# Daniel-Starr/pointcloudhookup

Hardware: AMD Instinct MI355X
Metric: Mpts/s ground-filter+tower-cluster, 100 M-pt corridor; % HBM roofline on kNN (higher is better)
Workload: dtype f32 (filter) + f64 (distance predicate)

## Files before the change

### pointcloudhookup_amd/csrc/pch_dbscan.hip

```cpp
#include "pch_prims.h"

namespace pch {

constexpr int DB_THREADS = 256;
constexpr int DB_WAVES   = DB_THREADS / 64;
constexpr int DB_ROWS    = 25;
constexpr int INT_BIG    = 0x7fffffff;
constexpr int DB_FEW_QUERIES = 24;
constexpr int DB_AHEAD = 3;
constexpr long long DB_LONG_TOT = 8192;
constexpr int DB_SEGS = 43;

struct DbGrid {
    float   ox, oy, oz;
    double  cell;
    double  inv_cell;
    double  eps2;
    float   eps2_lo, eps2_hi;
    int     bx, by, bz;
    int     mx, my, mz;
    int64_t chunk_size;
    const uint32_t* chunk_bad;
    const uint32_t* chunk_cells;
    int     min_samples;
// ... 411 lines not shown
        float4 nxt[CS_ROUNDS];
        auto tile = [&](int t0, auto FULL_T) {
            constexpr bool FULL = decltype(FULL_T)::value;
            float4 row[CS_ROUNDS];
            uint32_t key[CS_ROUNDS], rank[CS_ROUNDS];
            const int seg = t0 + w * (64 * CS_ROUNDS);
#pragma unroll
            for (int r = 0; r < CS_ROUNDS; ++r) row[r] = nxt[r];
            if (t0 + CS_TILE < cn) fetch(t0 + CS_TILE, nxt);
#ifdef PCH_CS_STAMPS
            tlast = wall_clock64();
#endif
#pragma unroll
            for (int r = 0; r < CS_ROUNDS; ++r) {
                const bool valid = FULL || seg + r * 64 + l < cn;
                bool ok;
                key[r] = cs_cell_key(g, row[r].x, row[r].y, row[r].z, ok);
                const uint32_t d = (relkey(key[r]) >> shift) & mask;
                uint32_t np;
                const uint32_t rk = dbits <= 8 ? wave_match<8>(d, valid, np) : wave_match<9>(d, valid, np);
                const uint32_t prior = cnt[w][d];
                __builtin_amdgcn_wave_barrier();
                if (valid && rk == 0) cnt[w][d] = prior + np;
                __builtin_amdgcn_wave_barrier();
                rank[r] = prior + rk;
            }
            __syncthreads();
            CS_TILE_STAMP(0);
            if (tid < CS_BINS) {
                uint32_t run = base[tid];
#pragma unroll
                for (int w2 = 0; w2 < CS_WAVES; ++w2) {
                    const uint32_t cc = cnt[w2][tid];
                    off[w2][tid] = run;
                    cnt[w2][tid] = 0;
                    run += cc;
                }
                base[tid] = run;
            }
            __syncthreads();
            CS_TILE_STAMP(1);
#pragma unroll
            for (int r = 0; r < CS_ROUNDS; ++r) {
                if (FULL || seg + r * 64 + l < cn) {
                    const uint32_t d = (relkey(key[r]) >> shift) & mask;
                    const uint32_t pos = off[w][d] + rank[r];
                    dst[pos] = row[r];
                    if constexpr (LAST) keys_out[lo + pos] = hi | key[r];
                }
            }
            CS_TILE_STAMP(2);
        };
        fetch(0, nxt);
        int t0 = 0;
        for (; t0 + CS_TILE <= cn; t0 += CS_TILE) tile(t0, std::true_type{});
        if (t0 < cn) tile(t0, std::false_type{});
        __syncthreads();
        CS_STAMP();
    };
    for (int p = 0; p < passes; ++p) {
        const bool first = p == 0, last = p == passes - 1;
        if (first && last) run_pass(p, std::true_type{}, std::true_type{});
        else if (first)    run_pass(p, std::true_type{}, std::false_type{});
        else if (last)     run_pass(p, std::false_type{}, std::true_type{});
        else               run_pass(p, std::false_type{}, std::false_type{});
    }
#ifdef PCH_CS_STAMPS
    __syncthreads();
    CS_STAMP();
    if (stamps && blockIdx.x == gridDim.x / 2 && threadIdx.x == 0) for (int k = 0; k < 3; ++k) stamps[8 + k] = tacc[k];
#endif
}

constexpr int CT_SLOTS = 4096;
constexpr int CT_BITS  = 12;
constexpr int CT_CELLS = 1024;
constexpr uint32_t CT_EMPTY = 0xFFFFFFFFu;
static_assert(CT_SLOTS == 1 << CT_BITS && CT_CELLS + CS_THREADS < CT_SLOTS, "the table never fills (see sweep 1)");

__device__ __forceinline__ uint32_t ct_hash(uint32_t k) { return (k * 0x9E3779B1u) >> (32 - CT_BITS); }

__global__ __launch_bounds__(CS_THREADS) void db_cellscatter_k(
    const float* __restrict__ xyz, int64_t n, DbGrid g, uint32_t* __restrict__ bad, uint32_t* __restrict__ ovf,
    float4* __restrict__ pts, uint64_t* __restrict__ keys_out, uint32_t* __restrict__ status) {
    __shared__ uint32_t tkey[CT_SLOTS];
    __shared__ uint32_t tcnt[CT_SLOTS];
    __shared__ uint32_t skey[CT_CELLS];
    __shared__ uint32_t wsum[CS_WAVES];
    __shared__ uint32_t flags[5];
    const int tid = threadIdx.x, w = wave_id(), l = lane_id();
    const int64_t c = blockIdx.x;
    const int64_t lo = c * g.chunk_size;
    const int cn = (int)((n - lo) < g.chunk_size ? (n - lo) : g.chunk_size);
    const Row3* __restrict__ rows = reinterpret_cast<const Row3*>(xyz) + lo;
    for (int j = tid; j < CT_SLOTS; j += CS_THREADS) { tkey[j] = CT_EMPTY; tcnt[j] = 0u; }
    if (tid < 5) flags[tid] = 0u;
    __syncthreads();
    constexpr int HU = 8;
    for (int i0 = 0; i0 < cn; i0 += HU * CS_THREADS) {
        if (__hip_atomic_load(&flags[3], __ATOMIC_RELAXED, __HIP_MEMORY_SCOPE_WORKGROUP)) break;
        Row3 q[HU];
#pragma unroll
        for (int u = 0; u < HU; ++u) {
            const int i = i0 + u * CS_THREADS + tid;
            q[u] = rows[i < cn ? i : 0];
        }
#pragma unroll
        for (int u = 0; u < HU; ++u) {
            const bool in = i0 + u * CS_THREADS + tid < cn;
            const bool fin = fabsf(q[u].x) < INFINITY && fabsf(q[u].y) < INFINITY && fabsf(q[u].z) < INFINITY;
            bool ok;
            const uint32_t k = cs_cell_key(g, q[u].x, q[u].y, q[u].z, ok);
            if (in && !fin) flags[0] = 1u;
            else if (in && !ok) flags[1] = 1u;
            if (in && fin && __hip_atomic_load(&flags[3], __ATOMIC_RELAXED, __HIP_MEMORY_SCOPE_WORKGROUP) == 0u) {
                uint32_t h = ct_hash(k);
                for (int p = 0; p < CT_SLOTS; ++p, h = (h + 1u) & (CT_SLOTS - 1)) {
                    const uint32_t old = atomicCAS(&tkey[h], CT_EMPTY, k);
                    if (old == CT_EMPTY && atomicAdd(&flags[2], 1u) >= (uint32_t)CT_CELLS) flags[3] = 1u;
                    if (old == CT_EMPTY || old == k) { atomicAdd(&tcnt[h], 1u); break; }
                }
            }
        }
    }
    __syncthreads();
    const bool isbad = flags[0] != 0u;
    const uint32_t ncell = flags[2];
    const bool over = !isbad && ncell > (uint32_t)CT_CELLS;
    if (tid == 0) {
        ovf[c] = over ? 1u : 0u;
        if (!over) {
            bad[c] = isbad ? 1u : 0u;
            if (!isbad && flags[1]) atomicOr(status, 1u);
        }
    }
    if (over) return;
    const int sh = g.bx + g.by + g.bz;
    const uint64_t hi = sh < 64 ? ((uint64_t)c << sh) : 0ull;
    if (isbad || ncell == 1u) {
        for (int i = tid; i < cn; i += CS_THREADS) {
            const Row3 q = rows[i];
            float4 o4;
            o4.x = q.x; o4.y = q.y; o4.z = q.z; o4.w = __uint_as_float((uint32_t)(lo + i));
            pts[lo + i] = o4;
            bool ok;
            keys_out[lo + i] = isbad ? hi : (hi | cs_cell_key(g, q.x, q.y, q.z, ok));
        }
        return;
    }
    const int P = 1 << (32 - __clz((int)ncell - 1));
    for (int j0 = 0; j0 < CT_SLOTS; j0 += CS_THREADS) {
        const uint32_t k = tkey[j0 + tid];
        const uint64_t m = __ballot(k != CT_EMPTY);
        uint32_t base = 0;
        if (l == 0 && m) base = atomicAdd(&flags[4], (uint32_t)__popcll(m));
        base = (uint32_t)__shfl((int)base, 0, 64);
        if (k != CT_EMPTY) skey[base + (uint32_t)__popcll(m & lanemask_lt())] = k;
    }
    for (int j = (int)ncell + tid; j < P; j += CS_THREADS) skey[j] = CT_EMPTY;
    __syncthreads();
    for (int k = 2; k <= P; k <<= 1) {
        for (int j = k >> 1; j > 0; j >>= 1) {
            for (int t = tid; t < P / 2; t += CS_THREADS) {
                const int a = 2 * t - (t & (j - 1)), b = a + j;
                const uint32_t ka = skey[a], kb = skey[b];
                if ((ka > kb) == ((a & k) == 0)) { skey[a] = kb; skey[b] = ka; }
            }
            __syncthreads();
        }
    }
    {
        uint32_t slot[4], cnt[4], sum = 0;
#pragma unroll
        for (int u = 0; u < 4; ++u) {
            const int j = 4 * tid + u;
            slot[u] = 0; cnt[u] = 0;
            if (j < (int)ncell) {
                const uint32_t k = skey[j];
                uint32_t h = ct_hash(k);
                for (int p = 0; p < CT_SLOTS && tkey[h] != k; ++p) h = (h + 1u) & (CT_SLOTS - 1);
                slot[u] = h;
                cnt[u] = tcnt[h];
            }
            sum += cnt[u];
        }
        const uint32_t incl = wave_scan_incl(sum);
        if (l == 63) wsum[w] = incl;
        __syncthreads();
        uint32_t run = incl - sum;
        for (int w2 = 0; w2 < w; ++w2) run += wsum[w2];
#pragma unroll
        for (int u = 0; u < 4; ++u) {
            if (4 * tid + u < (int)ncell) tcnt[slot[u]] = run;
            run += cnt[u];
        }
    }
    __syncthreads();
    for (int i0 = 0; i0 < cn; i0 += HU * CS_THREADS) {
        Row3 q[HU];
#pragma unroll
        for (int u = 0; u < HU; ++u) {
            const int i = i0 + u * CS_THREADS + tid;
            q[u] = rows[i < cn ? i : 0];
        }
#pragma unroll
        for (int u = 0; u < HU; ++u) {
            const int i = i0 + u * CS_THREADS + tid;
            if (i < cn) {
                bool ok;
                const uint32_t k = cs_cell_key(g, q[u].x, q[u].y, q[u].z, ok);
                uint32_t h = ct_hash(k);
                for (int p = 0; p < CT_SLOTS && tkey[h] != k; ++p) h = (h + 1u) & (CT_SLOTS - 1);
                const uint32_t pos = atomicAdd(&tcnt[h], 1u);
                if (pos >= (uint32_t)cn) continue;
                float4 o4;
                o4.x = q[u].x; o4.y = q[u].y; o4.z = q[u].z; o4.w = __uint_as_float((uint32_t)(lo + i));
                pts[lo + pos] = o4;
                keys_out[lo + pos] = hi | k;
            }
        }
    }
}

constexpr int DC_ITEMS = SCAN_TILE / DB_THREADS;
static_assert(DC_ITEMS == 8, "two 64-byte key loads per thread");

__device__ __forceinline__ void dc_load_keys(const uint64_t* __restrict__ keys, int64_t base, int64_t n,
                                             uint64_t (&k)[DC_ITEMS], uint64_t& prev) {
    if (base + DC_ITEMS <= n) {
        const ulonglong2* q = reinterpret_cast<const ulonglong2*>(keys + base);
#pragma unroll
        for (int j = 0; j < DC_ITEMS / 2; ++j) { const ulonglong2 v = q[j]; k[2 * j] = v.x; k[2 * j + 1] = v.y; }
    } else {
#pragma unroll
        for (int j = 0; j < DC_ITEMS; ++j) k[j] = base + j < n ? keys[base + j] : 0ull;
    }
    prev = (base > 0 && base < n) ? keys[base - 1] : 0ull;
}

__global__ __launch_bounds__(DB_THREADS) void db_heads_k(const uint64_t* __restrict__ keys, int64_t n,
                                                         uint32_t* __restrict__ tile_sums) {
    __shared__ uint32_t wsum[DB_WAVES];
    const int64_t base = (int64_t)blockIdx.x * SCAN_TILE + (int64_t)threadIdx.x * DC_ITEMS;
    uint64_t k[DC_ITEMS], prev;
    dc_load_keys(keys, base, n, k, prev);
    uint32_t heads = 0;
#pragma unroll
    for (int j = 0; j < DC_ITEMS; ++j) {
        const int64_t i = base + j;
        heads += (i < n && (i == 0 || k[j] != (j ? k[j - 1] : prev))) ? 1u : 0u;
    }
    heads = wave_reduce_add(heads);
    if (lane_id() == 0) wsum[wave_id()] = heads;
    __syncthreads();
    if (threadIdx.x == 0) {
        uint32_t t = 0;
#pragma unroll
        for (int w = 0; w < DB_WAVES; ++w) t += wsum[w];
        tile_sums[blockIdx.x] = t;
    }
}

__global__ __launch_bounds__(DB_THREADS) void db_cells_k(const uint64_t* __restrict__ keys,
                                                         const uint32_t* __restrict__ tile_excl, int64_t n,
                                                         int sh, int64_t nchunks,
                                                         uint32_t* __restrict__ cid,
                                                         uint32_t* __restrict__ cell_start,
                                                         uint64_t* __restrict__ cell_key,
                                                         uint32_t* __restrict__ chunk_cells,
                                                         uint32_t* __restrict__ cell_acc) {
    __shared__ uint32_t wsum[DB_WAVES];
    const int64_t base = (int64_t)blockIdx.x * SCAN_TILE + (int64_t)threadIdx.x * DC_ITEMS;
    uint64_t k[DC_ITEMS], prev;
    dc_load_keys(keys, base, n, k, prev);
    bool hd[DC_ITEMS];
    uint32_t heads = 0;
// ... 18 lines not shown
            const uint64_t key = k[j], pk = j ? k[j - 1] : prev;
            cell_start[cc[j]] = (uint32_t)i;
            cell_key[cc[j]] = key;
            uint4* a4 = reinterpret_cast<uint4*>(cell_acc + 8 * (int64_t)cc[j]);
            a4[0] = make_uint4(0u, 0u, 0u, 0u);
            a4[1] = make_uint4(0u, 0u, 0u, 0u);
            const uint64_t ch = sh < 64 ? key >> sh : 0, pch = sh < 64 ? pk >> sh : 0;
            if (i == 0 || ch != pch) chunk_cells[ch] = cc[j];
        }
        if (i == n - 1) { cell_start[cc[j] + 1] = (uint32_t)n; chunk_cells[nchunks] = cc[j] + 1; }
    }
    if (base + DC_ITEMS <= n) {
        uint4* o = reinterpret_cast<uint4*>(cid + base);
        o[0] = make_uint4(cc[0], cc[1], cc[2], cc[3]);
        o[1] = make_uint4(cc[4], cc[5], cc[6], cc[7]);
    } else {
#pragma unroll
        for (int j = 0; j < DC_ITEMS; ++j)
            if (base + j < n) cid[base + j] = cc[j];
    }
}
struct RowSet {
    int ca[DB_ROWS], cb[DB_ROWS];
};

__device__ __forceinline__ int db_lower(const uint64_t* __restrict__ a, int m, uint64_t k) {
    int lo = 0, hi = m;
    while (lo < hi) { const int mid = (lo + hi) >> 1; if (a[mid] < k) lo = mid + 1; else hi = mid; }
    return lo;
}
__device__ __forceinline__ int2 db_row_run(const DbGrid& g, const uint64_t* __restrict__ cell_key, uint64_t key,
                                           int row) {
    const uint64_t cx = key & ((1ull << g.bx) - 1);
    const uint64_t cy = (key >> g.bx) & ((1ull << g.by) - 1);
    const uint64_t cz = (key >> (g.bx + g.by)) & ((1ull << g.bz) - 1);
    const int sh = g.bx + g.by + g.bz;
    const uint64_t chunk = sh < 64 ? (key >> sh) : 0;
    const int ny = (int)cy + DB_ROW_DY[row], nz = (int)cz + DB_ROW_DZ[row];
    int2 v;
    v.x = 0; v.y = 0;
    if (ny >= 0 && ny <= g.my && nz >= 0 && nz <= g.mz) {
        const int xlo = (int)cx - 2 < 0 ? 0 : (int)cx - 2;
        const int xhi = (int)cx + 2 > g.mx ? g.mx : (int)cx + 2;
        const int c0 = (int)g.chunk_cells[chunk], c1 = (int)g.chunk_cells[chunk + 1];
        v.x = c0 + db_lower(cell_key + c0, c1 - c0, db_pack(g, chunk, (uint64_t)nz, (uint64_t)ny, (uint64_t)xlo));
        const uint64_t khi = db_pack(g, chunk, (uint64_t)nz, (uint64_t)ny, (uint64_t)xhi);
        uint64_t kk[5];
#pragma unroll
        for (int i = 0; i < 5; ++i) kk[i] = v.x + i < c1 ? cell_key[v.x + i] : ~0ull;
        int cntx = 0;
#pragma unroll
        for (int i = 0; i < 5; ++i) cntx += kk[i] <= khi ? 1 : 0;
        v.y = v.x + cntx;
    }
    return v;
}

__device__ __forceinline__ void db_rows(const DbGrid& g, const uint64_t* __restrict__ cell_key, uint64_t key,
                                        RowSet* __restrict__ rs, const int2* __restrict__ rowtab, int cell) {
    const int l = lane_id();
    if (rowtab) {
        if (l < DB_ROWS) {
            const int2 v = rowtab[(int64_t)cell * DB_ROWS + l];
            rs->ca[l] = v.x;
            rs->cb[l] = v.y;
        }
        __builtin_amdgcn_wave_barrier();
        return;
    }
    if (l < DB_ROWS) {
        const int2 v = db_row_run(g, cell_key, key, l);
        rs->ca[l] = v.x;
        rs->cb[l] = v.y;
    }
    __builtin_amdgcn_wave_barrier();
}

__global__ __launch_bounds__(DB_THREADS) void db_rowtab_k(DbGrid g, const uint64_t* __restrict__ cell_key,
                                                          int m, int2* __restrict__ rowtab) {
    const int c = (blockIdx.x * DB_WAVES + wave_id()) * 2 + (lane_id() >> 5);
    const int l = lane_id() & 31;
    if (c >= m || l >= DB_ROWS) return;
    rowtab[(int64_t)c * DB_ROWS + l] = db_row_run(g, cell_key, cell_key[c], l);
}

template <bool COUNT>
__global__ __launch_bounds__(DB_THREADS) void db_core_k(DbGrid g, const float4* __restrict__ pts,
                                                        const uint32_t* __restrict__ cell_start,
                                                        const uint64_t* __restrict__ cell_key, int m,
                                                        const int2* __restrict__ rowtab,
                                                        uint8_t* __restrict__ core_s,
                                                        uint32_t* __restrict__ cell_ncore,
                                                        unsigned long long* __restrict__ stats) {
    unsigned long long n_useful = 0, n_slots = 0, n_tiles = 0;
    auto tally = [&]() {
        if (COUNT && lane_id() == 0) {
            atomicAdd(&stats[0], n_useful); atomicAdd(&stats[1], n_slots);
            atomicAdd(&stats[2], 1ull); atomicAdd(&stats[3], n_tiles);
        }
    };
    __shared__ RowSet rows[DB_WAVES];
    __shared__ DbPair tiles[DB_WAVES][32];
    __shared__ uint32_t seg_a[DB_WAVES][DB_SEGS], seg_b[DB_WAVES][DB_SEGS];
    const int c = blockIdx.x * DB_WAVES + wave_id();
    if (c >= m) return;
    const int l = lane_id();
    const uint32_t s = cell_start[c], e = cell_start[c + 1];
    const int cnt = (int)(e - s);
    {
        const int sh = g.bx + g.by + g.bz;
        if (g.chunk_bad[sh < 64 ? (cell_key[c] >> sh) : 0]) {
            for (uint32_t i = s + l; i < e; i += 64) core_s[i] = 0;
            if (l == 0) cell_ncore[c] = 0;
            return;
        }
    }
    if (cnt >= g.min_samples) {
        for (uint32_t i = s + l; i < e; i += 64) core_s[i] = 1;
        if (l == 0) cell_ncore[c] = (uint32_t)cnt;
        return;
    }
    RowSet* rs = &rows[wave_id()];
    db_rows(g, cell_key, cell_key[c], rs, rowtab, c);
    long long tot = 0;
    if (l < DB_ROWS) tot = (long long)cell_start[rs->cb[l]] - (long long)cell_start[rs->ca[l]];
    tot = wave_reduce_add(tot);
    if (tot < (long long)g.min_samples) {
        for (uint32_t i = s + l; i < e; i += 64) core_s[i] = 0;
        if (l == 0) cell_ncore[c] = 0;
        return;
    }
    uint32_t* sa = seg_a[wave_id()];
    uint32_t* sb = seg_b[wave_id()];
    {
        const uint64_t xmask = (1ull << g.bx) - 1;
        const int cx = (int)(cell_key[c] & xmask);
        if (l < DB_ROWS) {
            const int ca = rs->ca[l], cb = rs->cb[l];
            if (l < 9) {
                int ia = ca, ib = cb;
                if (ca < cb) {
                    if ((int)(cell_key[ca] & xmask) == cx - 2) ia = ca + 1;
                    if (ib > ia && (int)(cell_key[cb - 1] & xmask) == cx + 2) ib = cb - 1;
                }
                sa[l] = cell_start[ia];      sb[l] = cell_start[ib];
                sa[9 + l] = cell_start[ca];  sb[9 + l] = cell_start[ia];
                sa[18 + l] = cell_start[ib]; sb[18 + l] = cell_start[cb];
            } else {
                sa[18 + l] = cell_start[ca]; sb[18 + l] = cell_start[cb];
            }
        }
        __builtin_amdgcn_wave_barrier();
    }
    uint32_t ncore = 0;
    const bool long_sweep = tot >= DB_LONG_TOT;
    if (cnt < DB_FEW_QUERIES) {
        for (uint32_t q = s; q < e; ++q) {
            const float4 qp = pts[q];
            int count = 0;
            if (long_sweep) {
                for (int r = 0; r < DB_SEGS && count < g.min_samples; ++r) {
                    const uint32_t pa = sa[r], pb = sb[r];
                    for (uint32_t j0 = pa; j0 < pb && count < g.min_samples; j0 += 64u * DB_AHEAD) {
                        float4 P[DB_AHEAD];
#pragma unroll
                        for (int u = 0; u < DB_AHEAD; ++u) {
// ... 797 lines not shown
        }
    }
}

__global__ __launch_bounds__(DB_THREADS) void db_remap_points_k(const float4* __restrict__ pts,
                                                                const uint8_t* __restrict__ core_s, int64_t n,
                                                                const int32_t* __restrict__ map, int32_t nmap,
                                                                int32_t* __restrict__ labels) {
    const int64_t i = (int64_t)blockIdx.x * DB_THREADS + threadIdx.x;
    if (i >= n) return;
    const uint32_t o = __float_as_uint(pts[i].w);
    int32_t lab = -1;
    if (core_s[i]) {
        const int32_t old = labels[o];
        lab = (old >= 0 && old < nmap) ? map[old] : -1;
    }
    labels[o] = lab;
}
__global__ __launch_bounds__(DB_THREADS) void db_remap_cells_k(int* __restrict__ cell_label,
                                                               const uint32_t* __restrict__ cell_ncore, int m,
                                                               const int32_t* __restrict__ map, int32_t nmap) {
    const int c = blockIdx.x * DB_THREADS + threadIdx.x;
    if (c >= m) return;
    if (cell_ncore[c] == 0) return;
    const int old = cell_label[c];
    const int neu = (old >= 0 && old < nmap) ? map[old] : -1;
    cell_label[c] = neu >= 0 ? neu : INT_BIG;
}

__global__ __launch_bounds__(DB_THREADS) void db_first_rows_k(const uint32_t* __restrict__ bits,
                                                              const uint32_t* __restrict__ rank, int64_t nw,
                                                              int32_t* __restrict__ out) {
    const int64_t i = (int64_t)blockIdx.x * DB_THREADS + threadIdx.x;
    if (i >= nw) return;
    uint32_t b = bits[i];
    uint32_t c = rank[i];
    while (b) {
        const int t = __builtin_ctz(b);
        b &= b - 1;
        out[c++] = (int32_t)(i * 32 + t);
    }
}

__global__ __launch_bounds__(DB_THREADS) void db_strip_pairs_k(const float4* __restrict__ pts,
                                                               const uint32_t* __restrict__ cell_start,
                                                               const uint8_t* __restrict__ core_s,
                                                               const uint32_t* __restrict__ cell_ncore,
                                                               const float* __restrict__ cell_box,
                                                               const int* __restrict__ cell_label, int m, float x_lo,
                                                               float x_hi, int32_t cap, int32_t* __restrict__ out_pairs,
                                                               int32_t* __restrict__ out_count) {
    const int c = blockIdx.x * DB_WAVES + wave_id();
    if (c >= m) return;
    if (cell_ncore[c] == 0) return;
    if (!(cell_box[6 * (int64_t)c + 3] >= x_lo && cell_box[6 * (int64_t)c] < x_hi)) return;
    const int l = lane_id();
    const uint32_t a = cell_start[c], b = cell_start[c + 1];
    uint32_t best = 0xFFFFFFFFu;
    for (uint32_t i = a + l; i < b; i += 64) {
        if (!core_s[i]) continue;
        const float4 p = pts[i];
        if (p.x >= x_lo && p.x < x_hi) {
            const uint32_t row = __float_as_uint(p.w);
            best = row < best ? row : best;
        }
    }
    best = wave_reduce_min(best);
    if (l == 0 && best != 0xFFFFFFFFu) {
        const int32_t slot = atomicAdd(out_count, 1);
        if (slot < cap) {
            out_pairs[2 * slot] = (int32_t)best;
            out_pairs[2 * slot + 1] = cell_label[c];
        }
    }
}

__global__ void db_prelabel_k(const uint32_t* __restrict__ total, int32_t* __restrict__ out_nclusters,
                              uint32_t* __restrict__ box_acc, int64_t box_words) {
    if (threadIdx.x == 0 && blockIdx.x == 0) *out_nclusters = (int32_t)*total;
    const int64_t i = (int64_t)blockIdx.x * blockDim.x + threadIdx.x;
    if (box_acc && i < box_words) box_acc[i] = 0u;
}

struct DbWs {
    uint32_t* meta;
    uint64_t *k0, *k1, *cell_key;
    uint32_t *v0, *v1, *head, *cid, *cell_start, *cell_ncore, *flag, *radix_ws, *scan_ws;
    float4   *pts, *xbuf;
    uint8_t*  core_s;
    float*    cell_box;
    uint32_t* cell_acc;
    int*      cell_min;
    int      *parent, *root, *comp_min, *cell_label;
    int2*     rowtab;
    int64_t   rowtab_cells;
    uint32_t* chunk_bad;
    uint32_t* chunk_ovf;
    uint32_t* chunk_cells;
    uint32_t* comp;
    uint32_t* flag2;
    unsigned long long* core_stats;
    uint32_t* scan1_b;
};

static void db_plan(Arena& a, int64_t n, DbWs& w) {
    const int64_t nn = n > 0 ? n : 1;
    w.meta = a.take<uint32_t>(64);
    w.scan1_b = a.take<uint32_t>(scan1_ws_u32(nn / 32 + 1));
    w.chunk_cells = a.take<uint32_t>(nn + 8);
    w.core_stats = a.take<unsigned long long>(4);
    w.chunk_bad = a.take<uint32_t>(nn + 8);
    w.chunk_ovf = a.take<uint32_t>(nn + 8);
    w.k0 = a.take<uint64_t>(nn);
    w.k1 = a.take<uint64_t>(nn);
    w.v0 = a.take<uint32_t>(nn);
    w.v1 = a.take<uint32_t>(nn);
    w.head = a.take<uint32_t>(nn + 8);
    w.cid = a.take<uint32_t>(nn);
    w.pts = a.take<float4>(nn);
    w.xbuf = a.take<float4>(nn);
    w.core_s = a.take<uint8_t>(nn);
    w.cell_key = a.take<uint64_t>(nn);
    w.cell_start = a.take<uint32_t>(nn + 8);
    w.cell_ncore = a.take<uint32_t>(nn);
    w.cell_box = a.take<float>(6 * nn);
    w.cell_acc = a.take<uint32_t>(8 * nn);
    w.cell_min = a.take<int>(nn);
    w.parent = a.take<int>(nn);
    w.root = a.take<int>(nn);
    w.comp_min = a.take<int>(nn);
    w.cell_label = a.take<int>(nn);
    w.flag = a.take<uint32_t>(nn / 16 + 256);
    w.radix_ws = a.take<uint32_t>(radix_ws_u32(nn));
    w.scan_ws = a.take<uint32_t>(scan_ws_u32(nn));
    w.rowtab_cells = nn / 4 > 65536 ? nn / 4 : (nn < 65536 ? nn : 65536);
    w.rowtab = a.take<int2>((size_t)w.rowtab_cells * DB_ROWS);
    w.comp = a.take<uint32_t>(3 * nn);
    w.flag2 = a.take<uint32_t>(nn + 8);
}

struct DbCells {
    DbGrid g; const float4* pts; const uint32_t* cell_start; const uint64_t* cell_key; int m;
    const int2* rowtab;
    const uint8_t* core_s; const uint32_t* cell_ncore; const float* cell_box;
};
#define DB_GRID_ARGS(c) (c).g, (c).pts, (c).cell_start, (c).cell_key, (c).m, (c).rowtab
#define DB_CELL_ARGS(c) DB_GRID_ARGS(c), (c).core_s, (c).cell_ncore, (c).cell_box

struct DbTuning { int sort_mode; bool no_boxfold, no_xcd, count_pairs; };
static int g_sort_mode = -1;
static thread_local bool g_count_pairs = false;
static DbTuning db_tuning() {
    static const bool no_boxfold = getenv("PCH_DB_NO_BOXFOLD") != nullptr, no_xcd = getenv("PCH_DB_NO_XCD") != nullptr;
    int m = __atomic_load_n(&g_sort_mode, __ATOMIC_RELAXED);
    if (m < 0) {
        const char* e = getenv("PCH_DBSCAN_SORT");
        m = (e && strcmp(e, "chunk") == 0) ? 1 : (e && strcmp(e, "global") == 0) ? 2 : 0;
        __atomic_store_n(&g_sort_mode, m, __ATOMIC_RELAXED);
    }
    return {m, no_boxfold, no_xcd, g_count_pairs};
}

struct DbLastRun { void* ws; size_t ws_bytes; int64_t n; DbCells c; };
static thread_local DbLastRun g_last = {nullptr, 0, 0, {}};

void ws_touched(const void* base, size_t bytes) {
// ... 76 lines not shown
    g.eps2_lo = nextafterf((float)(g.eps2 * (1.0 - 1.0 / 1048576.0)), -INFINITY);
    g.eps2_hi = nextafterf((float)(g.eps2 * (1.0 + 1.0 / 1048576.0)), INFINITY);
    if (!(g.eps2_hi < 3.0e38f)) { g.eps2_lo = -1.0f; g.eps2_hi = NAN; }
    g.chunk_size = r.chunk_size;
    g.chunk_bad = r.w.chunk_bad;
    g.chunk_cells = r.w.chunk_cells;
    g.min_samples = min_samples;
    int mc[3] = {0, 0, 0};
    bool overflow = false;
    for (int k = 0; k < 3; ++k) {
        const double ext = ((double)box[3 + k] - (double)box[k]) * g.inv_cell;
        if (!(ext < 2.0e9)) overflow = true;
        else mc[k] = (int)ext + 1;
    }
    cellbits = db_cell_bits(g, mc[0], mc[1], mc[2]);
    nbits = cellbits + bits_for((uint64_t)r.nchunks);
    return overflow || nbits > 64;
}

static int db_run_chunks(const DbRun& r, double eps, int32_t min_samples, void* ws, size_t ws_bytes, int32_t* k_host) {
    int32_t offset = 0;
    for (int64_t c = 0; c < r.nchunks; ++c) {
        const int64_t lo = c * r.chunk_size, cn = (r.n - lo) < r.chunk_size ? (r.n - lo) : r.chunk_size;
        int32_t kc = 0;
        PCH_TRY(dbscan_run(r.xyz + 3 * lo, cn, eps, min_samples, 0, nullptr, r.labels + lo,
                           r.core ? r.core + lo : nullptr, r.out_nclusters, ws, ws_bytes, r.s, &kc));
        if (kc > 0 && offset > 0)
            PCH_LAUNCH("db_add_offset", db_add_offset_k, dim3((unsigned)ceil_div(cn, DB_THREADS)), dim3(DB_THREADS), 0,
                       r.s, r.labels + lo, cn, offset);
        offset += kc;
    }
    PCH_HIP_TRY(hipMemcpyAsync(r.out_nclusters, &offset, sizeof(int32_t), hipMemcpyHostToDevice, r.s));
    PCH_HIP_TRY(hipStreamSynchronize(r.s));
    if (k_host) *k_host = offset;
    g_last.ws = nullptr;
    return PCH_OK;
}

static int db_compress(const DbRun& r, DbGrid& g, int& cellbits, bool& done) {
    const DbWs& w = r.w; const hipStream_t s = r.s; const int64_t n = r.n;
    const unsigned gn = (unsigned)ceil_div(n, DB_THREADS);
    int64_t* first_bad = reinterpret_cast<int64_t*>(w.meta + 12);
    PCH_HIP_TRY(hipMemsetAsync(first_bad, 0xFF, sizeof(int64_t), s));
    PCH_LAUNCH("db_first_bad", db_first_bad_k, dim3(db_stride_blocks(n)), dim3(DB_THREADS), 0, s, r.xyz, n,
               reinterpret_cast<unsigned long long*>(first_bad));
    PCH_HIP_TRY(hipMemsetAsync(w.meta + 6, 0, 6 * sizeof(uint32_t), s));
    for (int axis = 0; axis < 3; ++axis) {
        PCH_LAUNCH("dbc_axis_keys", dbc_axis_keys_k, dim3(gn), dim3(DB_THREADS), 0, s, r.xyz, n, axis, w.k0, w.v0);
        PCH_TRY(radix_sort_pairs(w.k0, w.v0, w.k1, w.v1, n, 32, w.radix_ws, s));
        const bool in1 = radix_sort_result_buffer(32) == 1;
        const uint64_t* ksa = in1 ? w.k1 : w.k0;
        const uint32_t* vsa = in1 ? w.v1 : w.v0;
        PCH_LAUNCH("dbc_heads", dbc_heads_k, dim3(gn), dim3(DB_THREADS), 0, s, ksa, n, g.inv_cell, w.flag2);
        PCH_TRY(scan_exclusive_u32(w.flag2, w.head, n, w.scan_ws, nullptr, s));
        PCH_HIP_TRY(hipMemsetAsync(w.cell_start, 0, sizeof(uint32_t) * (size_t)(n + 8), s));
        for (int phase = 0; phase < 2; ++phase)
            PCH_LAUNCH("dbc_local", dbc_local_k, dim3(gn), dim3(DB_THREADS), 0, s, ksa, w.flag2, w.head, n, g.inv_cell,
                       w.cell_box, phase, w.cid, w.cell_start, w.meta + 6);
        PCH_TRY(scan_exclusive_u32(w.cell_start, w.cell_start, n, w.scan_ws, nullptr, s));
        PCH_LAUNCH("dbc_comp", dbc_comp_k, dim3(gn), dim3(DB_THREADS), 0, s, vsa, w.flag2, w.head, w.cid, w.cell_start,
                   n, axis, w.comp, w.meta + 9);
    }
    uint32_t back[8];
    PCH_HIP_TRY(hipMemcpyAsync(back, w.meta + 6, sizeof(back), hipMemcpyDeviceToHost, s));
    PCH_HIP_TRY(hipStreamSynchronize(s));
    int64_t bad_row;
    memcpy(&bad_row, &back[6], sizeof(bad_row));
    if (bad_row >= 0) {
        PCH_TRY(db_all_noise(r));
        g_last.ws = nullptr;
        done = true;
        return PCH_OK;
    }
    if (back[0] != 0) { set_error("compressed cell coordinates out of range"); return PCH_ERR_RANGE; }
    cellbits = db_cell_bits(g, (int)back[3], (int)back[4], (int)back[5]);
    if (cellbits > 64) {
        set_error("cell key needs %d bits even with compressed coordinates (%lld isolated points?)", cellbits, (long long)n);
        return PCH_ERR_RANGE;
    }
    return PCH_OK;
}

static int db_sorted_keys(const DbRun& r, const DbGrid& g, int cellbits, int nbits, bool compressed, int sort_mode,
                          const uint64_t*& ks) {
    const DbWs& w = r.w; const hipStream_t s = r.s; const int64_t n = r.n, nchunks = r.nchunks;
    const unsigned gn = (unsigned)ceil_div(n, DB_THREADS);
    const size_t bytes = (size_t)(reinterpret_cast<char*>(w.chunk_cells + nchunks + 1) - reinterpret_cast<char*>(w.meta + 4));
    PCH_HIP_TRY(hipMemsetAsync(w.meta + 4, 0, (bytes + 15) & ~size_t(15), s));
    if (!compressed && cellbits <= 31 && r.chunk_size <= CS_MAX_CHUNK && sort_mode != 2 &&
        (sort_mode == 1 || nchunks >= CS_MIN_CHUNKS)) {
        PCH_LAUNCH("db_cellscatter", db_cellscatter_k, dim3((unsigned)nchunks), dim3(CS_THREADS), 0, s, r.xyz, n, g,
                   w.chunk_bad, w.chunk_ovf, w.pts, w.k1, w.meta + 6);
        PCH_LAUNCH("db_chunksort", db_chunksort_k, dim3((unsigned)nchunks), dim3(CS_THREADS), 0, s, r.xyz, n, g,
                   w.chunk_ovf, w.chunk_bad, w.xbuf, w.pts, w.k1, w.meta + 6, (unsigned long long*)w.cell_box);
#ifdef PCH_CS_STAMPS
        {
            unsigned long long t[11];
            PCH_HIP_TRY(hipStreamSynchronize(s));
            PCH_HIP_TRY(hipMemcpy(t, w.cell_box, sizeof(t), hipMemcpyDeviceToHost));
            for (int q = 1; q <= 6; ++q)
                fprintf(stderr, "chunksort phase %d: %.2f us\n", q, (double)(long long)(t[q] - t[q - 1]) / 100.0);
            fprintf(stderr, "chunksort tiles: rank %.2f us, offsets %.2f us, scatter %.2f us\n", (double)t[8] / 100.0,
                    (double)t[9] / 100.0, (double)t[10] / 100.0);
        }
#endif
        ks = w.k1;
        return PCH_OK;
    }
    PCH_HIP_TRY(hipMemsetAsync(w.chunk_bad, 0, sizeof(uint32_t) * (size_t)(nchunks + 1), s));
    if (compressed) {
        PCH_LAUNCH("db_keys_comp", db_keys_comp_k, dim3(gn), dim3(DB_THREADS), 0, s, w.comp, n, g, w.k0, w.v0);
    } else {
        PCH_LAUNCH("db_chunkbad", db_chunkbad_k, dim3(db_stride_blocks(n)), dim3(DB_THREADS), 0, s, r.xyz, n,
                   r.chunk_size, w.chunk_bad);
        PCH_LAUNCH("db_keys", db_keys_k, dim3(gn), dim3(DB_THREADS), 0, s, r.xyz, n, g, w.chunk_bad, w.k0, w.v0,
                   w.meta + 6);
    }
    PCH_TRY(radix_sort_pairs(w.k0, w.v0, w.k1, w.v1, n, nbits, w.radix_ws, s));
    const bool in1 = radix_sort_result_buffer(nbits) == 1;
    ks = in1 ? w.k1 : w.k0;
    PCH_LAUNCH("db_gather", db_gather_k, dim3(gn), dim3(DB_THREADS), 0, s, r.xyz, ks, in1 ? w.v1 : w.v0, n, w.pts);
    return PCH_OK;
}

static int db_cells_core(const DbRun& r, const DbGrid& g, int cellbits, const uint64_t* ks, bool count_pairs,
                         DbCells& c) {
    const DbWs& w = r.w; const hipStream_t s = r.s; const int64_t n = r.n;
    const int64_t ntile = ceil_div(n, (int64_t)SCAN_TILE);
    PCH_LAUNCH("db_heads", db_heads_k, dim3((unsigned)ntile), dim3(DB_THREADS), 0, s, ks, n, w.scan_ws);
    PCH_TRY(scan_tile_sums_u32(w.scan_ws, ntile, w.meta + 7, s));
    uint32_t st_m[2];
    PCH_TRY(peek_enqueue(w.meta + 6, sizeof(st_m), s));
    PCH_LAUNCH("db_cells", db_cells_k, dim3((unsigned)ntile), dim3(DB_THREADS), 0, s, ks, w.scan_ws, n, cellbits,
               r.nchunks, w.cid, w.cell_start, w.cell_key, w.chunk_cells, w.cell_acc);
    PCH_TRY(peek_wait(st_m, sizeof(st_m)));
    if (st_m[0] != 0) {
        set_error("finite coordinates outside the supplied bounding box");
        return PCH_ERR_ARG;
    }
    const int m = (int)st_m[1];
    const unsigned gc = (unsigned)ceil_div(m, DB_WAVES);
    c = {g, w.pts, w.cell_start, w.cell_key, m, m <= w.rowtab_cells ? w.rowtab : nullptr, w.core_s, w.cell_ncore,
         w.cell_box};
    if (c.rowtab)
        PCH_LAUNCH("db_rowtab", db_rowtab_k, dim3((unsigned)ceil_div(m, 2 * DB_WAVES)), dim3(DB_THREADS), 0, s, g,
                   w.cell_key, m, w.rowtab);
    if (count_pairs) {
        PCH_HIP_TRY(hipMemsetAsync(w.core_stats, 0, 4 * sizeof(unsigned long long), s));
        PCH_LAUNCH("db_core_counting", db_core_k<true>, dim3(gc), dim3(DB_THREADS), 0, s, DB_GRID_ARGS(c), w.core_s,
                   w.cell_ncore, w.core_stats);
    } else {
        PCH_LAUNCH("db_core", db_core_k<false>, dim3(gc), dim3(DB_THREADS), 0, s, DB_GRID_ARGS(c), w.core_s,
                   w.cell_ncore, nullptr);
    }
    PCH_LAUNCH("db_cellstats", db_cellstats_k, dim3((unsigned)ceil_div(n, (int64_t)DB_WAVES * 64 * DB_CS_ROUNDS)),
               dim3(DB_THREADS), 0, s, w.pts, w.cid, w.core_s, n, w.cell_acc, w.flag, ceil_div(n, 32));
    PCH_LAUNCH("db_cellfin", db_cellfin_k, dim3((unsigned)ceil_div(m, DB_THREADS)), dim3(DB_THREADS), 0, s,
               w.cell_acc, m, w.cell_box, w.cell_min, w.parent, w.comp_min);
    return PCH_OK;
}

static int db_union(const DbRun& r, const DbCells& c) {
    const DbWs& w = r.w; const hipStream_t s = r.s; const int m = c.m;
    const unsigned gc = (unsigned)ceil_div(m, DB_WAVES);
    const uint8_t* face_todo = nullptr;
    if (c.rowtab) {
        PCH_LAUNCH("db_union_pairs", db_union_pairs_k, dim3((unsigned)ceil_div(4 * (int64_t)m, DB_THREADS)),
                   dim3(DB_THREADS), 0, s, DB_CELL_ARGS(c), w.parent, reinterpret_cast<uint8_t*>(w.root));
        face_todo = reinterpret_cast<const uint8_t*>(w.root);
    }
    PCH_LAUNCH("db_union0", db_union_face_k, dim3(gc), dim3(DB_THREADS), 0, s, DB_CELL_ARGS(c), w.parent, face_todo);
    PCH_LAUNCH("db_flatten", db_flatten_k, dim3((unsigned)ceil_div(m, DB_THREADS)), dim3(DB_THREADS), 0, s,
               w.parent, m);
    PCH_LAUNCH("db_union1", db_union_k, dim3(gc), dim3(DB_THREADS), 0, s, DB_CELL_ARGS(c), w.parent);
    PCH_LAUNCH("db_compmin", db_compmin_k, dim3((unsigned)ceil_div(m, DB_THREADS)), dim3(DB_THREADS), 0, s,
               w.cell_min, w.cell_ncore, m, w.parent, w.root, w.comp_min);
    return PCH_OK;
}

static int db_labels(const DbRun& r, const DbCells& c, const DbTuning& tune, int32_t* k_host, DbBoxOut* boxes) {
    const DbWs& w = r.w; const hipStream_t s = r.s; const int64_t n = r.n, nchunks = r.nchunks; const int m = c.m;
    const int64_t nw = ceil_div(n, 32);
    uint32_t* bits = w.flag;
    uint32_t* wrank = w.flag + ((nw + 63) & ~int64_t(63));
    static_assert(DB_CS_ROUNDS * 64 * DB_WAVES / DB_THREADS <= 32, "db_cellstats_k's grid has a thread per bitmap word");
    PCH_LAUNCH("db_mark", db_mark_k, dim3((unsigned)ceil_div(m, DB_THREADS)), dim3(DB_THREADS), 0, s,
               w.root, w.comp_min, m, bits);
    if (scan1_pays(nw)) PCH_TRY(scan1_exclusive_popc_u32(bits, wrank, nw, w.scan1_b, w.meta + 8, s));
    else PCH_TRY(scan_exclusive_popc_u32(bits, wrank, nw, w.scan_ws, w.meta + 8, s));
    uint32_t* box_acc = (boxes && boxes->acc && boxes->cap > 0 && !tune.no_boxfold) ? boxes->acc : nullptr;
    const int32_t box_cap = box_acc ? boxes->cap : 0;
    PCH_LAUNCH("db_prelabel", db_prelabel_k, dim3((unsigned)(box_acc ? ceil_div(8 * (int64_t)box_cap, 256) : 1)),
               dim3(256), 0, s, w.meta + 8, r.out_nclusters, box_acc, 8 * (int64_t)box_cap);
    if (k_host) PCH_TRY(peek_enqueue(r.out_nclusters, sizeof(int32_t), s));
    const int bpc = (nchunks >= 16 && !tune.no_xcd) ? (int)ceil_div(r.chunk_size, DB_LAB_TILE) : 0;
    const unsigned gl = bpc > 0 ? (unsigned)(8 * ceil_div(nchunks, 8) * bpc) : (unsigned)ceil_div(n, DB_LAB_TILE);
    PCH_LAUNCH("db_label", db_label_k, dim3(gl), dim3(DB_THREADS), 0, s, w.pts, w.cid, w.core_s, w.root, w.comp_min,
               bits, wrank, n, w.cell_start, w.cell_label, r.labels, r.core, r.chunk_size, bpc, nchunks, box_acc,
               box_cap);
    PCH_LAUNCH("db_border", db_border_k, dim3((unsigned)ceil_div(m, DB_WAVES)), dim3(DB_THREADS), 0, s,
               DB_CELL_ARGS(c), w.cell_label, r.labels, box_acc, box_cap);
    if (box_acc) boxes->done = true;
    if (k_host) {
        PCH_TRY(peek_wait(k_host, sizeof(int32_t)));
        if (*k_host < 0) {
            set_error("stage C: a device-side look-back wait ran out of its budget; outputs are undefined");
            return PCH_ERR_TIMEOUT;
        }
    }
    return PCH_OK;
}

}

using namespace pch;

extern "C" int pch_first_nonfinite_row_f32(const float* xyz, int64_t n, int64_t* out_row, void* stream) {
    PCH_DEVICE_GUARD(out_row);
    hipStream_t s = (hipStream_t)stream;
    PCH_REQUIRE(n >= 0 && out_row && (n == 0 || xyz), "bad argument");
    PCH_HIP_TRY(hipMemsetAsync(out_row, 0xFF, sizeof(int64_t), s));
    if (n == 0) return PCH_OK;
    PCH_LAUNCH("db_first_bad", db_first_bad_k, dim3(db_stride_blocks(n)), dim3(DB_THREADS), 0, s, xyz, n,
               reinterpret_cast<unsigned long long*>(out_row));
    return PCH_OK;
}

extern "C" void pch_dbscan_set_sort_mode(int mode) {
    __atomic_store_n(&g_sort_mode, (mode == 1 || mode == 2) ? mode : 0, __ATOMIC_RELAXED);
}

extern "C" size_t pch_dbscan_ws_bytes(int64_t n) {
    if (n < 0) return 0;
    Arena a;
    DbWs w;
    db_plan(a, n, w);
    return a.off;
}

int pch::dbscan_run(const float* xyz, int64_t n, double eps, int32_t min_samples, int64_t chunk_size,
                    const float* aabb_host, int32_t* labels, uint8_t* core, int32_t* out_nclusters, void* ws,
                    size_t ws_bytes, hipStream_t s, int32_t* k_host, DbBoxOut* boxes) {
    if (k_host) *k_host = 0;
    if (boxes) boxes->done = false;
    PCH_REQUIRE(n >= 0 && n < (int64_t(1) << 31), "n out of range [0, 2^31)");
    PCH_REQUIRE(eps > 0.0, "eps must be > 0 (sklearn: InvalidParameterError)");
    PCH_REQUIRE(min_samples >= 1, "min_samples must be >= 1 (sklearn: InvalidParameterError)");
    PCH_REQUIRE(out_nclusters != nullptr, "out_nclusters is null");
    if (n == 0) {
        PCH_HIP_TRY(hipMemsetAsync(out_nclusters, 0, sizeof(int32_t), s));
        return PCH_OK;
    }
    PCH_REQUIRE(xyz && labels && ws, "null buffer");
    Arena a(ws, ws_bytes);
    DbWs w;
    db_plan(a, n, w);
    if (a.overflow) { set_error("workspace too small: need %zu bytes", a.off); return PCH_ERR_WORKSPACE; }
    if (chunk_size <= 0 || chunk_size > n) chunk_size = n;
    const DbRun r = {xyz, n, chunk_size, ceil_div(n, chunk_size), labels, core, out_nclusters, s, w};
    const DbTuning tune = db_tuning();

    float box[6];
    bool done = false;
    PCH_TRY(db_bounds(r, aabb_host, box, done));
    if (done) return PCH_OK;
    DbGrid g;
    int cellbits, nbits;
    const bool overflow = db_grid(r, box, eps, min_samples, g, cellbits, nbits);
    if (overflow) {
        if (r.nchunks > 1) return db_run_chunks(r, eps, min_samples, ws, ws_bytes, k_host);
        PCH_TRY(db_compress(r, g, cellbits, done));
        if (done) return PCH_OK;
        nbits = cellbits;
    }
    const uint64_t* ks;
    DbCells c;
    PCH_TRY(db_sorted_keys(r, g, cellbits, nbits, overflow, tune.sort_mode, ks));
    PCH_TRY(db_cells_core(r, g, cellbits, ks, tune.count_pairs, c));
    PCH_TRY(db_union(r, c));
    PCH_TRY(db_labels(r, c, tune, k_host, boxes));
    g_last = {ws, ws_bytes, n, c};
    return PCH_OK;
}

extern "C" int pch_dbscan_first_core_rows_i32(int64_t n, int32_t* out_rows, void* ws, size_t ws_bytes, void* stream) {
    PCH_DEVICE_GUARD(out_rows ? (const void*)out_rows : (const void*)ws);
    PCH_REQUIRE(n >= 0, "bad argument");
    if (n == 0) return PCH_OK;
    DbWs w;
    PCH_TRY(db_continue(__func__, n, ws, ws_bytes, w));
    PCH_REQUIRE(out_rows != nullptr, "null output");
    const int64_t nw = ceil_div(n, 32);
    const uint32_t* bits = w.flag;
    const uint32_t* wrank = w.flag + ((nw + 63) & ~int64_t(63));
    PCH_LAUNCH("db_first_rows", db_first_rows_k, dim3((unsigned)ceil_div(nw, DB_THREADS)), dim3(DB_THREADS), 0,
               (hipStream_t)stream, bits, wrank, nw, out_rows);
    return PCH_OK;
}

extern "C" void pch_dbscan_set_pair_counting(int enable) { g_count_pairs = enable != 0; }

extern "C" int pch_dbscan_pair_stats(int64_t n, uint64_t* out4_host, void* ws, size_t ws_bytes, void* stream) {
    PCH_DEVICE_GUARD(ws);
    PCH_REQUIRE(n >= 0 && out4_host, "bad argument");
    memset(out4_host, 0, 4 * sizeof(uint64_t));
    if (n == 0) return PCH_OK;
    DbWs w;
    PCH_TRY(db_continue(__func__, n, ws, ws_bytes, w));
    PCH_HIP_TRY(hipMemcpyAsync(out4_host, w.core_stats, 4 * sizeof(uint64_t), hipMemcpyDeviceToHost, (hipStream_t)stream));
    PCH_HIP_TRY(hipStreamSynchronize((hipStream_t)stream));
    return PCH_OK;
}

extern "C" int pch_dbscan_strip_pairs_i32(int64_t n, float x_lo, float x_hi, int32_t cap, int32_t* out_pairs,
                                          int32_t* out_count, void* ws, size_t ws_bytes, void* stream) {
    PCH_DEVICE_GUARD(out_count);
    hipStream_t s = (hipStream_t)stream;
    PCH_REQUIRE(n >= 0 && cap >= 0 && out_count && (cap == 0 || out_pairs), "bad argument");
    PCH_HIP_TRY(hipMemsetAsync(out_count, 0, sizeof(int32_t), s));
    if (n == 0 || !(x_lo < x_hi)) return PCH_OK;
    DbWs w;
    PCH_TRY(db_continue(__func__, n, ws, ws_bytes, w));
    const int m = g_last.c.m;
    PCH_LAUNCH("db_strip_pairs", db_strip_pairs_k, dim3((unsigned)ceil_div(m, DB_WAVES)), dim3(DB_THREADS), 0, s,
               w.pts, w.cell_start, w.core_s, w.cell_ncore, w.cell_box, w.cell_label, m, x_lo, x_hi, cap, out_pairs,
               out_count);
    return PCH_OK;
}

extern "C" int pch_dbscan_relabel_i32(const int32_t* map, int32_t nmap, int64_t n, int32_t* labels, void* ws,
                                      size_t ws_bytes, void* stream) {
    PCH_DEVICE_GUARD(labels);
    hipStream_t s = (hipStream_t)stream;
    PCH_REQUIRE(n >= 0 && nmap >= 0 && (nmap == 0 || map) && (n == 0 || labels), "bad argument");
    if (n == 0) return PCH_OK;
    DbWs w;
    PCH_TRY(db_continue(__func__, n, ws, ws_bytes, w));
    const DbCells& c = g_last.c;
    PCH_LAUNCH("db_remap_points", db_remap_points_k, dim3((unsigned)ceil_div(n, DB_THREADS)), dim3(DB_THREADS), 0, s,
               w.pts, w.core_s, n, map, nmap, labels);
    PCH_LAUNCH("db_remap_cells", db_remap_cells_k, dim3((unsigned)ceil_div(c.m, DB_THREADS)), dim3(DB_THREADS), 0, s,
               w.cell_label, w.cell_ncore, c.m, map, nmap);
    PCH_LAUNCH("db_border", db_border_k, dim3((unsigned)ceil_div(c.m, DB_WAVES)), dim3(DB_THREADS), 0, s,
               DB_CELL_ARGS(c), w.cell_label, labels, nullptr, 0);
    return PCH_OK;
}

extern "C" int pch_dbscan_f32(const float* xyz, int64_t n, double eps, int32_t min_samples,
                              int64_t chunk_size, const float* aabb_host, int32_t* labels,
                              uint8_t* core, int32_t* out_nclusters, void* ws, size_t ws_bytes,
                              void* stream) {
    PCH_DEVICE_GUARD(xyz ? (const void*)xyz : (const void*)out_nclusters);
    return dbscan_run(xyz, n, eps, min_samples, chunk_size, aabb_host, labels, core, out_nclusters, ws, ws_bytes,
                      (hipStream_t)stream, nullptr);
}
```

Before: 61110.

## Build cell table from per-chunk staged keys instead of rescanning sorted keys

The cell-scatter kernel now records each chunk's sorted distinct cell keys, their start offsets and the cell count per chunk. A new per-chunk kernel then builds cell_start, cell_key, cid and the row table straight from that compact data in LDS, using a prefix over chunk counts. This replaces the heads scan, tile-sum scan, cells kernel and separate rowtab kernel whenever no chunk overflowed. The old path stays as a fallback, chosen by a status word read back on the host. Each block recomputes the prefix over earlier chunks by looping over all of them, which is quadratic in the chunk count; the chunk cap of 4096 limits this cost.

```diff
diff --git a/pointcloudhookup_amd/csrc/pch_dbscan.hip b/pointcloudhookup_amd/csrc/pch_dbscan.hip
--- a/pointcloudhookup_amd/csrc/pch_dbscan.hip
+++ b/pointcloudhookup_amd/csrc/pch_dbscan.hip
@@ -517,7 +517,9 @@
 
 __global__ __launch_bounds__(CS_THREADS) void db_cellscatter_k(
     const float* __restrict__ xyz, int64_t n, DbGrid g, uint32_t* __restrict__ bad, uint32_t* __restrict__ ovf,
-    float4* __restrict__ pts, uint64_t* __restrict__ keys_out, uint32_t* __restrict__ status) {
+    float4* __restrict__ pts, uint64_t* __restrict__ keys_out, uint32_t* __restrict__ status,
+    uint32_t* __restrict__ stage_key, uint32_t* __restrict__ stage_pos, uint32_t* __restrict__ chunk_ncell,
+    uint32_t* __restrict__ cells) {
     __shared__ uint32_t tkey[CT_SLOTS];
     __shared__ uint32_t tcnt[CT_SLOTS];
     __shared__ uint32_t skey[CT_CELLS];
@@ -567,6 +569,11 @@
         if (!over) {
             bad[c] = isbad ? 1u : 0u;
             if (!isbad && flags[1]) atomicOr(status, 1u);
+            const uint32_t nc = isbad ? 1u : ncell;
+            chunk_ncell[c] = nc;
+            atomicAdd(&cells[0], nc);
+        } else {
+            atomicOr(&cells[1], 1u);
         }
     }
     if (over) return;
@@ -579,7 +586,9 @@
             o4.x = q.x; o4.y = q.y; o4.z = q.z; o4.w = __uint_as_float((uint32_t)(lo + i));
             pts[lo + i] = o4;
             bool ok;
-            keys_out[lo + i] = isbad ? hi : (hi | cs_cell_key(g, q.x, q.y, q.z, ok));
+            const uint32_t k = isbad ? 0u : cs_cell_key(g, q.x, q.y, q.z, ok);
+            keys_out[lo + i] = hi | k;
+            if (i == 0) { stage_key[lo] = k; stage_pos[lo] = 0u; }
         }
         return;
     }
@@ -626,7 +635,12 @@
         for (int w2 = 0; w2 < w; ++w2) run += wsum[w2];
 #pragma unroll
         for (int u = 0; u < 4; ++u) {
-            if (4 * tid + u < (int)ncell) tcnt[slot[u]] = run;
+            const int j = 4 * tid + u;
+            if (j < (int)ncell) {
+                tcnt[slot[u]] = run;
+                stage_key[lo + j] = skey[j];
+                stage_pos[lo + j] = run;
+            }
             run += cnt[u];
         }
     }
@@ -811,6 +825,92 @@
     const int l = lane_id() & 31;
     if (c >= m || l >= DB_ROWS) return;
     rowtab[(int64_t)c * DB_ROWS + l] = db_row_run(g, cell_key, cell_key[c], l);
+}
+
+constexpr int64_t DB_CELLTAB_MAX_CHUNKS = 4096;
+
+__device__ __forceinline__ int2 db_row_run_lds(const DbGrid& g, const uint32_t* skey, int nc, uint32_t key, int row,
+                                               int first) {
+    const uint32_t cx = key & ((1u << g.bx) - 1u);
+    const uint32_t cy = (key >> g.bx) & ((1u << g.by) - 1u);
+    const uint32_t cz = (key >> (g.bx + g.by)) & ((1u << g.bz) - 1u);
+    const int ny = (int)cy + DB_ROW_DY[row], nz = (int)cz + DB_ROW_DZ[row];
+    int2 v;
+    v.x = 0; v.y = 0;
+    if (ny >= 0 && ny <= g.my && nz >= 0 && nz <= g.mz) {
+        const int xlo = (int)cx - 2 < 0 ? 0 : (int)cx - 2;
+        const int xhi = (int)cx + 2 > g.mx ? g.mx : (int)cx + 2;
+        const uint32_t yz = (((uint32_t)nz << g.by) | (uint32_t)ny) << g.bx;
+        const uint32_t klo = yz | (uint32_t)xlo, khi = yz | (uint32_t)xhi;
+        int lo = 0, hi = nc;
+        while (lo < hi) { const int mid = (lo + hi) >> 1; if (skey[mid] < klo) lo = mid + 1; else hi = mid; }
+        int cntx = 0;
+#pragma unroll
+        for (int i = 0; i < 5; ++i) cntx += (lo + i < nc && skey[lo + i] <= khi) ? 1 : 0;
+        v.x = first + lo;
+        v.y = v.x + cntx;
+    }
+    return v;
+}
+
+__global__ __launch_bounds__(CS_THREADS) void db_celltab_k(
+    DbGrid g, int64_t n, int64_t nchunks, const uint32_t* __restrict__ stage_key,
+    const uint32_t* __restrict__ stage_pos, const uint32_t* __restrict__ chunk_ncell,
+    const uint32_t* __restrict__ cells, uint32_t* __restrict__ cell_start, uint64_t* __restrict__ cell_key,
+    uint32_t* __restrict__ chunk_cells, uint32_t* __restrict__ cell_acc, uint32_t* __restrict__ cid,
+    int2* __restrict__ rowtab, int64_t rowtab_cells) {
+    __shared__ uint32_t skey[CT_CELLS];
+    __shared__ uint32_t spos[CT_CELLS];
+    __shared__ uint32_t wsum[CS_WAVES];
+    if (cells[1] != 0u) return;
+    const int tid = threadIdx.x;
+    const int64_t c = blockIdx.x;
+    const int64_t lo = c * g.chunk_size;
+    uint32_t part = 0;
+    for (int64_t j = tid; j < c; j += CS_THREADS) part += chunk_ncell[j];
+    part = wave_reduce_add(part);
+    if (lane_id() == 0) wsum[wave_id()] = part;
+    const uint32_t ncc = chunk_ncell[c];
+    const int nc = (int)(ncc < (uint32_t)CT_CELLS ? ncc : (uint32_t)CT_CELLS);
+    for (int j = tid; j < nc; j += CS_THREADS) { skey[j] = stage_key[lo + j]; spos[j] = stage_pos[lo + j]; }
+    __syncthreads();
+    uint32_t first = 0;
+#pragma unroll
+    for (int w = 0; w < CS_WAVES; ++w) first += wsum[w];
+    const int64_t m = cells[0];
+    if ((int64_t)first + nc > m || m > n) return;
+    const int sh = g.bx + g.by + g.bz;
+    const uint64_t hi = sh < 64 ? ((uint64_t)c << sh) : 0ull;
+    for (int j = tid; j < nc; j += CS_THREADS) {
+        const int64_t cell = (int64_t)first + j;
+        cell_start[cell] = (uint32_t)(lo + spos[j]);
+        cell_key[cell] = hi | skey[j];
+        uint4* a4 = reinterpret_cast<uint4*>(cell_acc + 8 * cell);
+        a4[0] = make_uint4(0u, 0u, 0u, 0u);
+        a4[1] = make_uint4(0u, 0u, 0u, 0u);
+    }
+    if (tid == 0) {
+        chunk_cells[c] = first;
+        if (c == nchunks - 1) { chunk_cells[nchunks] = first + (uint32_t)nc; cell_start[(int64_t)first + nc] = (uint32_t)n; }
+    }
+    if (rowtab != nullptr && m <= rowtab_cells) {
+        for (int t = tid; t < nc * DB_ROWS; t += CS_THREADS) {
+            const int j = t / DB_ROWS;
+            rowtab[(int64_t)first * DB_ROWS + t] = db_row_run_lds(g, skey, nc, skey[j], t - j * DB_ROWS, (int)first);
+        }
+    }
+    const int cn = (int)((n - lo) < g.chunk_size ? (n - lo) : g.chunk_size);
+    const int share = ((cn + CS_WAVES - 1) / CS_WAVES + 63) & ~63;
+    const int p0 = wave_id() * share, p1 = p0 + share < cn ? p0 + share : cn;
+    int a = 0;
+    if (p0 + lane_id() < p1) {
+        int b = nc;
+        while (b - a > 1) { const int mid = (a + b) >> 1; if (spos[mid] <= (uint32_t)(p0 + lane_id())) a = mid; else b = mid; }
+    }
+    for (int p = p0 + lane_id(); p < p1; p += 64) {
+        while (a + 1 < nc && spos[a + 1] <= (uint32_t)p) ++a;
+        cid[lo + p] = first + (uint32_t)a;
+    }
 }
 
 template <bool COUNT>
@@ -1774,6 +1874,9 @@
     if (box_acc && i < box_words) box_acc[i] = 0u;
 }
 
+constexpr int DB_META_STATUS = 8, DB_META_M = 9, DB_META_OVF = 10, DB_META_K = 11;
+static_assert(DB_META_STATUS % 4 == 0 && DB_META_M == DB_META_STATUS + 1 && DB_META_OVF == DB_META_M + 1,
+              "the fill starts 16-byte aligned at the status word; status, m, overflow are read in one copy");
 struct DbWs {
     uint32_t* meta;
     uint64_t *k0, *k1, *cell_key;
@@ -2016,17 +2119,22 @@
 }
 
 static int db_sorted_keys(const DbRun& r, const DbGrid& g, int cellbits, int nbits, bool compressed, int sort_mode,
-                          const uint64_t*& ks) {
+                          const uint64_t*& ks, bool& staged) {
     const DbWs& w = r.w; const hipStream_t s = r.s; const int64_t n = r.n, nchunks = r.nchunks;
     const unsigned gn = (unsigned)ceil_div(n, DB_THREADS);
-    const size_t bytes = (size_t)(reinterpret_cast<char*>(w.chunk_cells + nchunks + 1) - reinterpret_cast<char*>(w.meta + 4));
-    PCH_HIP_TRY(hipMemsetAsync(w.meta + 4, 0, (bytes + 15) & ~size_t(15), s));
+    uint32_t* const fill = w.meta + DB_META_STATUS;
+    const size_t bytes = (size_t)(reinterpret_cast<char*>(w.chunk_cells + nchunks + 1) - reinterpret_cast<char*>(fill));
+    PCH_HIP_TRY(hipMemsetAsync(fill, 0, (bytes + 15) & ~size_t(15), s));
+    staged = false;
     if (!compressed && cellbits <= 31 && r.chunk_size <= CS_MAX_CHUNK && sort_mode != 2 &&
         (sort_mode == 1 || nchunks >= CS_MIN_CHUNKS)) {
         PCH_LAUNCH("db_cellscatter", db_cellscatter_k, dim3((unsigned)nchunks), dim3(CS_THREADS), 0, s, r.xyz, n, g,
-                   w.chunk_bad, w.chunk_ovf, w.pts, w.k1, w.meta + 6);
+                   w.chunk_bad, w.chunk_ovf, w.pts, w.k1, w.meta + DB_META_STATUS, w.v0, w.v1, w.head,
+                   w.meta + DB_META_M);
         PCH_LAUNCH("db_chunksort", db_chunksort_k, dim3((unsigned)nchunks), dim3(CS_THREADS), 0, s, r.xyz, n, g,
-                   w.chunk_ovf, w.chunk_bad, w.xbuf, w.pts, w.k1, w.meta + 6, (unsigned long long*)w.cell_box);
+                   w.chunk_ovf, w.chunk_bad, w.xbuf, w.pts, w.k1, w.meta + DB_META_STATUS,
+                   (unsigned long long*)w.cell_box);
+        staged = nchunks <= DB_CELLTAB_MAX_CHUNKS;
 #ifdef PCH_CS_STAMPS
         {
             unsigned long long t[11];
@@ -2048,7 +2156,7 @@
         PCH_LAUNCH("db_chunkbad", db_chunkbad_k, dim3(db_stride_blocks(n)), dim3(DB_THREADS), 0, s, r.xyz, n,
                    r.chunk_size, w.chunk_bad);
         PCH_LAUNCH("db_keys", db_keys_k, dim3(gn), dim3(DB_THREADS), 0, s, r.xyz, n, g, w.chunk_bad, w.k0, w.v0,
-                   w.meta + 6);
+                   w.meta + DB_META_STATUS);
     }
     PCH_TRY(radix_sort_pairs(w.k0, w.v0, w.k1, w.v1, n, nbits, w.radix_ws, s));
     const bool in1 = radix_sort_result_buffer(nbits) == 1;
@@ -2057,26 +2165,36 @@
     return PCH_OK;
 }
 
-static int db_cells_core(const DbRun& r, const DbGrid& g, int cellbits, const uint64_t* ks, bool count_pairs,
-                         DbCells& c) {
+static int db_cells_core(const DbRun& r, const DbGrid& g, int cellbits, const uint64_t* ks, bool staged,
+                         bool count_pairs, DbCells& c) {
     const DbWs& w = r.w; const hipStream_t s = r.s; const int64_t n = r.n;
-    const int64_t ntile = ceil_div(n, (int64_t)SCAN_TILE);
-    PCH_LAUNCH("db_heads", db_heads_k, dim3((unsigned)ntile), dim3(DB_THREADS), 0, s, ks, n, w.scan_ws);
-    PCH_TRY(scan_tile_sums_u32(w.scan_ws, ntile, w.meta + 7, s));
-    uint32_t st_m[2];
-    PCH_TRY(peek_enqueue(w.meta + 6, sizeof(st_m), s));
-    PCH_LAUNCH("db_cells", db_cells_k, dim3((unsigned)ntile), dim3(DB_THREADS), 0, s, ks, w.scan_ws, n, cellbits,
-               r.nchunks, w.cid, w.cell_start, w.cell_key, w.chunk_cells, w.cell_acc);
-    PCH_TRY(peek_wait(st_m, sizeof(st_m)));
-    if (st_m[0] != 0) {
+    uint32_t st[3] = {0u, 0u, 1u};
+    if (staged) {
+        PCH_TRY(peek_enqueue(w.meta + DB_META_STATUS, sizeof(st), s));
+        PCH_LAUNCH("db_celltab", db_celltab_k, dim3((unsigned)r.nchunks), dim3(CS_THREADS), 0, s, g, n, r.nchunks,
+                   w.v0, w.v1, w.head, w.meta + DB_META_M, w.cell_start, w.cell_key, w.chunk_cells, w.cell_acc, w.cid,
+                   w.rowtab, w.rowtab_cells);
+        PCH_TRY(peek_wait(st, sizeof(st)));
+    }
+    const bool from_keys = st[2] != 0u;
+    if (from_keys) {
+        const int64_t ntile = ceil_div(n, (int64_t)SCAN_TILE);
+        PCH_LAUNCH("db_heads", db_heads_k, dim3((unsigned)ntile), dim3(DB_THREADS), 0, s, ks, n, w.scan_ws);
+        PCH_TRY(scan_tile_sums_u32(w.scan_ws, ntile, w.meta + DB_META_M, s));
+        PCH_TRY(peek_enqueue(w.meta + DB_META_STATUS, 2 * sizeof(uint32_t), s));
+        PCH_LAUNCH("db_cells", db_cells_k, dim3((unsigned)ntile), dim3(DB_THREADS), 0, s, ks, w.scan_ws, n, cellbits,
+                   r.nchunks, w.cid, w.cell_start, w.cell_key, w.chunk_cells, w.cell_acc);
+        PCH_TRY(peek_wait(st, 2 * sizeof(uint32_t)));
+    }
+    if (st[0] != 0) {
         set_error("finite coordinates outside the supplied bounding box");
         return PCH_ERR_ARG;
     }
-    const int m = (int)st_m[1];
+    const int m = (int)st[1];
     const unsigned gc = (unsigned)ceil_div(m, DB_WAVES);
     c = {g, w.pts, w.cell_start, w.cell_key, m, m <= w.rowtab_cells ? w.rowtab : nullptr, w.core_s, w.cell_ncore,
          w.cell_box};
-    if (c.rowtab)
+    if (c.rowtab && from_keys)
         PCH_LAUNCH("db_rowtab", db_rowtab_k, dim3((unsigned)ceil_div(m, 2 * DB_WAVES)), dim3(DB_THREADS), 0, s, g,
                    w.cell_key, m, w.rowtab);
     if (count_pairs) {
@@ -2120,12 +2238,12 @@
     static_assert(DB_CS_ROUNDS * 64 * DB_WAVES / DB_THREADS <= 32, "db_cellstats_k's grid has a thread per bitmap word");
     PCH_LAUNCH("db_mark", db_mark_k, dim3((unsigned)ceil_div(m, DB_THREADS)), dim3(DB_THREADS), 0, s,
                w.root, w.comp_min, m, bits);
-    if (scan1_pays(nw)) PCH_TRY(scan1_exclusive_popc_u32(bits, wrank, nw, w.scan1_b, w.meta + 8, s));
-    else PCH_TRY(scan_exclusive_popc_u32(bits, wrank, nw, w.scan_ws, w.meta + 8, s));
+    if (scan1_pays(nw)) PCH_TRY(scan1_exclusive_popc_u32(bits, wrank, nw, w.scan1_b, w.meta + DB_META_K, s));
+    else PCH_TRY(scan_exclusive_popc_u32(bits, wrank, nw, w.scan_ws, w.meta + DB_META_K, s));
     uint32_t* box_acc = (boxes && boxes->acc && boxes->cap > 0 && !tune.no_boxfold) ? boxes->acc : nullptr;
     const int32_t box_cap = box_acc ? boxes->cap : 0;
     PCH_LAUNCH("db_prelabel", db_prelabel_k, dim3((unsigned)(box_acc ? ceil_div(8 * (int64_t)box_cap, 256) : 1)),
-               dim3(256), 0, s, w.meta + 8, r.out_nclusters, box_acc, 8 * (int64_t)box_cap);
+               dim3(256), 0, s, w.meta + DB_META_K, r.out_nclusters, box_acc, 8 * (int64_t)box_cap);
     if (k_host) PCH_TRY(peek_enqueue(r.out_nclusters, sizeof(int32_t), s));
     const int bpc = (nchunks >= 16 && !tune.no_xcd) ? (int)ceil_div(r.chunk_size, DB_LAB_TILE) : 0;
     const unsigned gl = bpc > 0 ? (unsigned)(8 * ceil_div(nchunks, 8) * bpc) : (unsigned)ceil_div(n, DB_LAB_TILE);
@@ -2209,8 +2327,9 @@
     }
     const uint64_t* ks;
     DbCells c;
-    PCH_TRY(db_sorted_keys(r, g, cellbits, nbits, overflow, tune.sort_mode, ks));
-    PCH_TRY(db_cells_core(r, g, cellbits, ks, tune.count_pairs, c));
+    bool staged;
+    PCH_TRY(db_sorted_keys(r, g, cellbits, nbits, overflow, tune.sort_mode, ks, staged));
+    PCH_TRY(db_cells_core(r, g, cellbits, ks, staged, tune.count_pairs, c));
     PCH_TRY(db_union(r, c));
     PCH_TRY(db_labels(r, c, tune, k_host, boxes));
     g_last = {ws, ws_bytes, n, c};
```

After: 62590, median of 6. +2.4%, better.
